# HeyWeCome/WhisprRec

Measured on AMD Instinct MI355X. Metric: BPR training triplets/sec, higher is better.
Workload: dtype f32; 1 GPU; BPRMF emb_size=64, synthetic 1000000 users x 1000000 items (uniform ids), batch 65536, SGD l2=0, plan build in timed region; batch=65536, emb_size=64, optimizer=SGD, plan_chunk_batches=64, tables=single GPU, step_stream=whisprrec_amd.hip_ops.PipelinedSgd, plan=group plan (no per-batch sort: flags + lists of the shared rows, wr_group.hip), chained_step_launch=True, plan_build=on a side stream, beside the steps of the chunk before

## Files before the change

whisprrec_amd/csrc/wr_group.hip:

```cpp
#include "wr_common.h"
#include <hip/hip_ext.h>

#include <algorithm>

namespace wr {

constexpr int kGpThreads = 1024;
constexpr unsigned kGpRangeBits = 18;
constexpr int kGpWords = 1 << (kGpRangeBits - 5);
constexpr int kGpCap = 8192;
constexpr int kGpBins = 4096;
constexpr int kGpMaxBin = 256;
constexpr int kGpMaxRanges = 8;
constexpr int64_t kGpMaxBatch = 1 << 17;
constexpr int kGpLongRun = 64;
constexpr int kGpMetaWords = 16;
#ifndef WR_GP_DBG
#define WR_GP_DBG 0
#endif

struct GroupLayout {
    int64_t nb, B, fw;
    int R_u, R_i, cap_u, cap_i;
    unsigned mask_u, mask_i, hbits_u, hbits_i;
    int64_t flags, ucnt, icnt, ul_row, ul_src, il_row, il_src, total;
    int64_t zero_words;
};

static inline int ranges_for(int64_t n_rows, unsigned *mask, unsigned *hbits, int *cap) {
    unsigned bits = kGpRangeBits;
    while (bits < kGpRangeBits + 3 && (int64_t(1) << bits) < n_rows) ++bits;
    *mask = (1u << bits) - 1u;
    *hbits = bits;
    const int R = 1 << (bits - kGpRangeBits);
    *cap = kGpCap;
    return R;
}

static bool group_layout(int64_t n, int64_t B, int64_t n_users, int64_t n_items, GroupLayout &L) {
    if (n <= 0 || n >= (int64_t(1) << 31) || B <= 0 || B > kGpMaxBatch) return false;
    if (n_users <= 0 || n_users >= (int64_t(1) << 31) || n_items <= 0 || n_items >= (int64_t(1) << 31)) return false;
    L.nb = (n + B - 1) / B;
    L.B = B;
    L.fw = (B + 31) / 32;
    L.R_u = ranges_for(n_users, &L.mask_u, &L.hbits_u, &L.cap_u);
    L.R_i = ranges_for(n_items, &L.mask_i, &L.hbits_i, &L.cap_i);
    L.flags = kGpMetaWords;
    L.ucnt = L.flags + L.nb * L.fw * 4;
    L.icnt = L.ucnt + align_up(L.nb * L.R_u, 4);
    L.zero_words = L.icnt + align_up(L.nb * L.R_i, 4);
    L.ul_row = L.zero_words;
    L.ul_src = L.ul_row + L.nb * L.R_u * (int64_t)L.cap_u;
    L.il_row = L.ul_src + L.nb * L.R_u * (int64_t)L.cap_u;
    L.il_src = L.il_row + L.nb * L.R_i * (int64_t)L.cap_i;
    L.total = L.il_src + L.nb * L.R_i * (int64_t)L.cap_i;
    return true;
}

struct GpDev {
    int *meta;
    unsigned *flags;
    int *ucnt, *icnt;
    int *ul_row, *ul_src, *il_row, *il_src;
    int R_u, R_i, cap_u, cap_i;
    unsigned mask_u, mask_i, hbits_u, hbits_i;
    int fw;
};

static inline GpDev group_dev(int32_t *plan, const GroupLayout &L) {
    return GpDev{plan, reinterpret_cast<unsigned *>(plan + L.flags), plan + L.ucnt, plan + L.icnt, plan + L.ul_row,
                 plan + L.ul_src, plan + L.il_row, plan + L.il_src, L.R_u, L.R_i, L.cap_u, L.cap_i, L.mask_u, L.mask_i,
                 L.hbits_u, L.hbits_i, (int)L.fw};
}

template <typename F>
__device__ __forceinline__ void gp_scan(const int *__restrict__ a, int cnt, F f) {
    if ((reinterpret_cast<uintptr_t>(a) & 15u) == 0) {
        const int n4 = cnt >> 2;
        const int4 *a4 = reinterpret_cast<const int4 *>(a);
        int i = threadIdx.x;
        for (; i + 3 * kGpThreads < n4; i += 4 * kGpThreads) {
            int4 v[4];
#pragma unroll
            for (int q = 0; q < 4; ++q) v[q] = a4[i + q * kGpThreads];
#pragma unroll
            for (int q = 0; q < 4; ++q) {
                const int at = 4 * (i + q * kGpThreads);
                f(v[q].x, at);
                f(v[q].y, at + 1);
                f(v[q].z, at + 2);
                f(v[q].w, at + 3);
            }
        }
        for (; i < n4; i += kGpThreads) {
            const int4 v = a4[i];
            f(v.x, 4 * i);
            f(v.y, 4 * i + 1);
            f(v.z, 4 * i + 2);
            f(v.w, 4 * i + 3);
        }
        for (int j = (n4 << 2) + threadIdx.x; j < cnt; j += kGpThreads) f(a[j], j);
    } else {
        for (int j = threadIdx.x; j < cnt; j += kGpThreads) f(a[j], j);
    }
}

__global__ __launch_bounds__(kGpThreads) void group_plan_kernel(const int *__restrict__ u, const int *__restrict__ p,
                                                                 const int *__restrict__ n, int64_t n_total, int B, int nb,
                                                                 int n_users, int n_items, GpDev L) {
    extern __shared__ __attribute__((aligned(16))) unsigned gp_lds[];
    unsigned *seen = gp_lds;
    unsigned long long *keys = reinterpret_cast<unsigned long long *>(gp_lds);
    unsigned *multi = gp_lds + 2 * kGpCap;
    unsigned *f0 = multi + kGpWords, *f1 = f0 + L.fw, *f2 = f1 + L.fw;
    int &n_list = *reinterpret_cast<int *>(f2 + L.fw);
    const int per = L.R_u + L.R_i;
    const unsigned lb = xcd_contiguous_id(blockIdx.x, gridDim.x);
    const int b = (int)(lb / (unsigned)per), rr = (int)(lb % (unsigned)per);
    const bool item = rr >= L.R_u;
    const unsigned r = (unsigned)(item ? rr - L.R_u : rr);
    const int64_t base = (int64_t)b * B;
    const int Bb = (int)((base + B <= n_total) ? B : (n_total - base));
    const unsigned n_rows = (unsigned)(item ? n_items : n_users);
    const unsigned mask = item ? L.mask_i : L.mask_u;
    const unsigned rb = (item ? L.hbits_i : L.hbits_u) - kGpRangeBits, rsel = (1u << rb) - 1u;
    for (int i = threadIdx.x; i < kGpWords; i += kGpThreads) {
        seen[i] = 0u;
        multi[i] = 0u;
    }
    for (int i = threadIdx.x; i < 3 * L.fw; i += kGpThreads) f0[i] = 0u;
    if (threadIdx.x == 0) n_list = 0;
    __syncthreads();
    auto mark = [&](int row, int) {
        if ((unsigned)row >= n_rows) {
            L.meta[0] = 1;
            return;
        }
        const unsigned h = (unsigned)row & mask;
        if ((h & rsel) != r) return;
        const unsigned bit = h >> rb, m = 1u << (bit & 31u);
        const unsigned old = atomicOr(&seen[bit >> 5], m);
        if (old & m) atomicOr(&multi[bit >> 5], m);
    };
    if (!(WR_GP_DBG & 8)) {
        if (item) {
            gp_scan(p + base, Bb, mark);
            gp_scan(n + base, Bb, mark);
        } else {
            gp_scan(u + base, Bb, mark);
        }
    }
    __syncthreads();
    auto several = [&](int row) -> bool {
        const unsigned h = (unsigned)row & mask;
        if ((h & rsel) != r) return false;
        const unsigned bit = h >> rb;
        return (multi[bit >> 5] >> (bit & 31u)) & 1u;
    };
    auto append = [&](int row, unsigned src) {
        const int pos = atomicAdd(&n_list, 1);
        if (pos < kGpCap) keys[pos] = ((unsigned long long)(unsigned)row << 32) | src;
    };
    if (!(WR_GP_DBG & 2)) {
        const bool next = b + 1 < nb && !(WR_GP_DBG & 16);
        const int64_t nbase = base + B;
        const int Bn = next ? (int)((nbase + B <= n_total) ? B : (n_total - nbase)) : 0;
        auto defer = [&](int row, int t) {
            if (several(row)) atomicOr(&f2[t >> 5], 1u << (t & 31));
        };
        if (item) {
            gp_scan(p + base, Bb, [&](int row, int t) {
                if (several(row)) {
                    atomicOr(&f0[t >> 5], 1u << (t & 31));
                    append(row, (unsigned)t << 1);
                }
            });
            gp_scan(n + base, Bb, [&](int row, int t) {
                if (several(row)) {
                    atomicOr(&f1[t >> 5], 1u << (t & 31));
                    append(row, ((unsigned)t << 1) | 1u);
                }
            });
            gp_scan(p + nbase, Bn, defer);
            gp_scan(n + nbase, Bn, defer);
        } else {
            gp_scan(u + base, Bb, [&](int row, int t) {
                if (several(row)) {
                    atomicOr(&f0[t >> 5], 1u << (t & 31));
                    append(row, (unsigned)t << 1);
                }
            });
            gp_scan(u + nbase, Bn, defer);
        }
    }
    __syncthreads();
    if (!(WR_GP_DBG & 4)) {
        unsigned *fb = L.flags + (int64_t)b * L.fw * 4;
        for (int w = threadIdx.x; w < L.fw; w += kGpThreads) {
            if (f0[w]) __hip_atomic_fetch_or(fb + 4 * w + (item ? 1 : 0), f0[w], __ATOMIC_RELAXED, __HIP_MEMORY_SCOPE_AGENT);
            if (item && f1[w]) __hip_atomic_fetch_or(fb + 4 * w + 2, f1[w], __ATOMIC_RELAXED, __HIP_MEMORY_SCOPE_AGENT);
            if (f2[w])
                __hip_atomic_fetch_or(fb + 4 * (L.fw + w) + 3, f2[w], __ATOMIC_RELAXED, __HIP_MEMORY_SCOPE_AGENT);
        }
    }
    const int cap = item ? L.cap_i : L.cap_u, R = item ? L.R_i : L.R_u;
    int m = n_list;
    if (m > cap) {
        if (threadIdx.x == 0) L.meta[1] = 1;
        m = cap;
    }
    int *cnt = reinterpret_cast<int *>(multi);
    unsigned short *out16 = reinterpret_cast<unsigned short *>(multi + kGpBins);
    int *wave_tot = reinterpret_cast<int *>(f0);
    auto bin_of = [&](unsigned long long k) -> int { return (int)(((((unsigned)(k >> 32)) & mask) >> rb) & (kGpBins - 1)); };
    int *lrow = (item ? L.il_row : L.ul_row) + ((int64_t)b * R + r) * cap, *lsrc = (item ? L.il_src : L.ul_src) + ((int64_t)b * R + r) * cap;
    __syncthreads();
    for (int i = threadIdx.x; i < kGpBins; i += kGpThreads) cnt[i] = 0;
    __syncthreads();
    if (!(WR_GP_DBG & 1)) {
        for (int j = threadIdx.x; j < m; j += kGpThreads) atomicAdd(&cnt[bin_of(keys[j])], 1);
        __syncthreads();
        constexpr int kOwn = kGpBins / kGpThreads;
        const int c0 = (int)threadIdx.x * kOwn;
        int local = 0;
#pragma unroll
        for (int j = 0; j < kOwn; ++j) local += cnt[c0 + j];
        int incl = local;
#pragma unroll
        for (int d = 1; d < 64; d <<= 1) {
            const int v = __shfl_up(incl, d, 64);
            if ((int)(threadIdx.x & 63) >= d) incl += v;
        }
        if ((threadIdx.x & 63) == 63) wave_tot[threadIdx.x >> 6] = incl;
        __syncthreads();
        int run = incl - local;
        for (int w = 0; w < (int)(threadIdx.x >> 6); ++w) run += wave_tot[w];
#pragma unroll
        for (int j = 0; j < kOwn; ++j) {
            const int c = cnt[c0 + j];
            cnt[c0 + j] = run;
            run += c;
        }
        __syncthreads();
        for (int j = threadIdx.x; j < m; j += kGpThreads) out16[atomicAdd(&cnt[bin_of(keys[j])], 1)] = (unsigned short)j;
        __syncthreads();
        for (int j = threadIdx.x; j < m; j += kGpThreads) {
            const unsigned long long k = keys[j];
            const int bin = bin_of(k);
            const int lo = bin ? cnt[bin - 1] : 0, hi = cnt[bin];
            if (hi - lo > kGpMaxBin) {
                L.meta[1] = 1;
                continue;
            }
            int pos = lo, same = 0;
            for (int jj = lo; jj < hi; ++jj) {
                const unsigned long long o = keys[out16[jj]];
                pos += o < k ? 1 : 0;
                same += (unsigned)(o >> 32) == (unsigned)(k >> 32) ? 1 : 0;
            }
            if (same > kGpLongRun) L.meta[2] = 1;
            lrow[pos] = (int)(k >> 32);
            lsrc[pos] = (int)(unsigned)k;
        }
    } else {
        for (int j = threadIdx.x; j < m; j += kGpThreads) {
            lrow[j] = (int)(keys[j] >> 32);
            lsrc[j] = (int)(unsigned)keys[j];
        }
    }
    if (threadIdx.x == 0) (item ? L.icnt : L.ucnt)[(int64_t)b * R + r] = m;
}

__global__ __launch_bounds__(kBlock) void narrow_ids_kernel(const int64_t *__restrict__ u, const int64_t *__restrict__ p,
                                                             const int64_t *__restrict__ n, int *__restrict__ u32,
                                                             int *__restrict__ p32, int *__restrict__ n32, int64_t cnt) {
    const int64_t i = (int64_t)blockIdx.x * kBlock + threadIdx.x;
    if (i >= cnt) return;
    const int64_t a = u[i], b = p[i], c = n[i];
    u32[i] = (a >= 0 && a < (int64_t(1) << 31)) ? (int)a : -1;
    p32[i] = (b >= 0 && b < (int64_t(1) << 31)) ? (int)b : -1;
    n32[i] = (c >= 0 && c < (int64_t(1) << 31)) ? (int)c : -1;
}

constexpr int kGsTile = 32;
constexpr int kGsAhead = 8;
constexpr int kGsShards = 64;
constexpr int kGsShardStride = 16;
constexpr int kGsStepWords = kGsShards * kGsShardStride;
constexpr int kGsDefChunk = 32;
constexpr int kGsLdsInts = 1024 + 8;
constexpr unsigned kGsSpinLimit = 1u << 22;

struct GsBatch {
    const int *u, *p, *n;
    const uint4 *flags;
    const int *ul_row, *ul_src, *ul_cnt, *il_row, *il_src, *il_cnt;
    int B, R_u, R_i, cap_u, cap_i;
};

struct GsArgs {
    float *U, *I;
    int D;
    float lr;
    GsBatch cur;
    float *Z, *ZU, *partials;
    float denom;
    GsBatch prev;
    const float *Zp, *ZUp, *partials_prev;
    int n_partials_prev;
    float denom_prev;
    float *loss_prev;
    int nA, nIT, nUT, nDS, tiles_at, side_at;
    int chained;
    unsigned *done, *timeout;
    float *Gs;
    int nL;
};

template <int NV>
__device__ __forceinline__ Row<NV> row_zero() {
    Row<NV> r;
#pragma unroll
    for (int k = 0; k < NV; ++k) r.v[k] = make_float4(0.f, 0.f, 0.f, 0.f);
    return r;
}

template <int T, int NV, bool FULL>
__device__ __forceinline__ void gs_single(const GsArgs &a, int t, int u, int p, int n, bool us, bool ps, bool ns, int lane,
                                          float &terms) {
    const Row<NV> ur = load_row<T, NV, FULL>(a.U, u, a.D, lane);
    const Row<NV> pr = load_row<T, NV, FULL>(a.I, p, a.D, lane);
    const Row<NV> nr = load_row<T, NV, FULL>(a.I, n, a.D, lane);
    const float sp = team_sum<T>(dot_partial<NV>(ur, pr));
    const float sn = team_sum<T>(dot_partial<NV>(ur, nr));
    float term, c;
    bpr_terms(sp, sn, a.denom, term, c);
    terms += term;
    Row<NV> g, z;
#pragma unroll
    for (int k = 0; k < NV; ++k) {
        g.v[k] = make_float4(c * (pr.v[k].x - nr.v[k].x), c * (pr.v[k].y - nr.v[k].y), c * (pr.v[k].z - nr.v[k].z),
                             c * (pr.v[k].w - nr.v[k].w));
        z.v[k] = make_float4(c * ur.v[k].x, c * ur.v[k].y, c * ur.v[k].z, c * ur.v[k].w);
    }
    const float lr = a.lr;
// ... 352 lines not shown
    TablePair tabs;
    const int32_t *u, *p, *n, *plan;
    int64_t n_triplets, batch_size, plan_words, workspace_bytes, sync_words;
    BatchRange range;
    float lr, *loss_out;
    void *const *events;
    void *workspace;
    uint32_t *sync;
    int n_cu;
    float *grad_slots;
    int64_t n_local_items, global_batch;
    hipStream_t stream;
};

template <int T, int NV, bool FULL>
static int32_t launch_group_steps(const GroupRun &g, const GroupLayout &L, const GpDev &G) {
    const int32_t D = g.tabs.D;
    const int64_t n_batches = g.range.n_batches, global_batch = g.global_batch;
    uint32_t *const sync = g.sync;
    const int64_t B = L.B;
    const int64_t ws_one = gs_ws_one(B, D), zb = align_up(B * (int64_t)D * 4, 256);
    char *ws = reinterpret_cast<char *>(g.workspace);
    float *Zs[2] = {reinterpret_cast<float *>(ws), reinterpret_cast<float *>(ws + ws_one)};
    float *ZUs[2] = {reinterpret_cast<float *>(ws + zb), reinterpret_cast<float *>(ws + ws_one + zb)};
    float *Ps[2] = {reinterpret_cast<float *>(ws + 2 * zb), reinterpret_cast<float *>(ws + ws_one + 2 * zb)};
    constexpr int TEAMS = kBlock / T;
    WR_HIP(hipMemsetAsync(sync, 0, (size_t)(n_batches * kGsStepWords) * 4, g.stream));
    uint32_t *timeout = sync + (g.sync_words - 4);
    int nDS = WR_GS_NDS;
    while (nDS > g.n_cu / 4 && nDS > 1) nDS >>= 1;
    auto batch_of = [&](int64_t b) {
        const int64_t off = b * B;
        const int Bk = (int)batch_len(g.n_triplets, B, b);
        return GsBatch{g.u + off, g.p + off, g.n + off, reinterpret_cast<const uint4 *>(G.flags + b * L.fw * 4),
                       G.ul_row + b * L.R_u * (int64_t)L.cap_u, G.ul_src + b * L.R_u * (int64_t)L.cap_u, G.ucnt + b * L.R_u,
                       G.il_row + b * L.R_i * (int64_t)L.cap_i, G.il_src + b * L.R_i * (int64_t)L.cap_i, G.icnt + b * L.R_i,
                       Bk, L.R_u, L.R_i, L.cap_u, L.cap_i};
    };
    auto ev = [&](int64_t k, int j) { return g.events ? reinterpret_cast<hipEvent_t>(g.events[2 * k + j]) : (hipEvent_t) nullptr; };
    int n_partials_prev = 0;
    for (int64_t k = 0; k <= n_batches; ++k) {
        GsArgs a{};
        a.U = g.tabs.U;
        a.I = g.tabs.I;
        a.D = D;
        a.lr = g.lr;
        a.done = sync + (k < n_batches ? k : 0) * kGsStepWords;
        a.timeout = timeout;
        a.Gs = g.grad_slots;
        a.nL = (int)g.n_local_items;
        const bool have_cur = k < n_batches, have_prev = k > 0;
        if (have_cur) {
            a.cur = batch_of(g.range.first_batch + k);
            a.Z = Zs[k & 1];
            a.ZU = ZUs[k & 1];
            a.partials = Ps[k & 1];
            a.denom = global_batch > 0 ? (float)global_batch : (float)a.cur.B;
            a.nA = (int)((a.cur.B + TEAMS - 1) / TEAMS);
            a.nDS = have_prev ? nDS : 0;
            a.chained = have_prev ? 1 : 0;
        }
        if (have_prev) {
            a.prev = batch_of(g.range.first_batch + k - 1);
            a.Zp = Zs[(k - 1) & 1];
            a.ZUp = ZUs[(k - 1) & 1];
            a.partials_prev = Ps[(k - 1) & 1];
            a.n_partials_prev = n_partials_prev;
            a.denom_prev = global_batch > 0 ? (float)global_batch : (float)a.prev.B;
            a.loss_prev = at_or_null(g.loss_out, k - 1);
            a.nIT = (int)std::min<int64_t>(WR_GS_NIT, (2 * B + kGsTile - 1) / kGsTile + L.R_i);
            a.nUT = (int)std::min<int64_t>(WR_GS_NUT, (B + kGsTile - 1) / kGsTile + L.R_u);
        }
        a.tiles_at = (int)((int64_t)a.nA * WR_GS_TILES_AT / 16);
        a.side_at = std::max(a.tiles_at, (int)((int64_t)a.nA * WR_GS_SIDE_AT / 16));
        const dim3 grid((unsigned)(a.nA + a.nIT + a.nUT + a.nDS));
        hipEvent_t e0 = have_cur ? ev(k, 0) : nullptr, e1 = have_cur ? ev(k, 1) : nullptr;
        if (e0 != nullptr || e1 != nullptr)
            hipExtLaunchKernelGGL((bprmf_group_step<T, NV, FULL>), grid, dim3(kBlock), 0, g.stream, e0, e1, 0, a);
        else
            hipLaunchKernelGGL((bprmf_group_step<T, NV, FULL>), grid, dim3(kBlock), 0, g.stream, a);
        WR_LAUNCH_CHECK("bprmf_group_step");
        n_partials_prev = a.nA + a.nDS;
    }
    return WR_OK;
}

static int32_t check_group_plan(const char *entry, const GroupRun &g, GroupLayout &L) {
    int32_t rc;
    if ((rc = check_whole_lines(entry, whole_lines(g.tabs.U, g.tabs.I, g.tabs.D), g.tabs.D)) != WR_OK) return rc;
    WR_REQUIRE(group_layout(g.n_triplets, g.batch_size, g.tabs.n_users, g.tabs.n_items, L), WR_E_RANGE,
               "group plan not applicable to n=%lld, batch=%lld", (long long)g.n_triplets, (long long)g.batch_size);
    WR_REQUIRE(g.plan_words >= L.total, WR_E_WORKSPACE, "group plan: %lld words < %lld", (long long)g.plan_words, (long long)L.total);
    return WR_OK;
}

static int32_t run_group(const char *entry, GroupRun &g, const GroupLayout &L, int64_t sync_batches) {
    int32_t rc;
    if ((rc = check_workspace(entry, g.workspace, g.workspace_bytes, 2 * gs_ws_one(g.batch_size, g.tabs.D))) != WR_OK) return rc;
    if ((rc = check_sync_words(entry, g.sync, g.sync_words, sync_batches * kGsStepWords + 4)) != WR_OK) return rc;
    if (g.range.n_batches == 0) return WR_OK;
    if (g.n_cu == 0 && (rc = device_cu_count(&g.n_cu)) != WR_OK) return rc;
    const GpDev G = group_dev(const_cast<int32_t *>(g.plan), L);
#define WR_CALL_GS(T_, NV_, FULL_) return launch_group_steps<T_, NV_, FULL_>(g, L, G)
    WR_DISPATCH_D(g.tabs.D, WR_CALL_GS);
#undef WR_CALL_GS
    return WR_OK;
}

}

using namespace wr;

extern "C" {

int64_t wr_group_plan_words(int64_t n_triplets, int64_t batch_size, int64_t n_users, int64_t n_items) {
    GroupLayout L;
    if (!group_layout(n_triplets, batch_size, n_users, n_items, L)) return 0;
    return L.total;
}

int32_t wr_group_plan_layout(int64_t n_triplets, int64_t batch_size, int64_t n_users, int64_t n_items, int64_t *out) {
    WR_REQUIRE(out != nullptr, WR_E_NULL, "out is NULL");
    GroupLayout L;
    WR_REQUIRE(group_layout(n_triplets, batch_size, n_users, n_items, L), WR_E_RANGE,
               "group plan not applicable to n=%lld, batch=%lld", (long long)n_triplets, (long long)batch_size);
    const int64_t v[16] = {L.nb, L.fw, L.R_u, L.R_i, (int64_t)L.mask_u, (int64_t)L.mask_i, L.flags, L.ucnt, L.icnt, L.ul_row,
                           L.ul_src, L.il_row, L.il_src, L.total, L.cap_u, L.cap_i};
    for (int i = 0; i < 16; ++i) out[i] = v[i];
    return WR_OK;
}

int32_t wr_narrow_ids_i64(const int64_t *u, const int64_t *p, const int64_t *n, int32_t *u32, int32_t *p32, int32_t *n32,
                          int64_t count, void *stream_) {
    WR_REQUIRE(u && p && n && u32 && p32 && n32, WR_E_NULL, "index arrays must not be NULL");
    WR_REQUIRE(count >= 0 && count < (int64_t(1) << 40), WR_E_SHAPE, "count out of range");
    if (count == 0) return WR_OK;
    hipLaunchKernelGGL(narrow_ids_kernel, dim3((unsigned)((count + kBlock - 1) / kBlock)), dim3(kBlock), 0,
                       reinterpret_cast<hipStream_t>(stream_), u, p, n, u32, p32, n32, count);
    WR_LAUNCH_CHECK("narrow_ids_kernel");
    return WR_OK;
}

int32_t wr_group_plan_build(const int32_t *u, const int32_t *p, const int32_t *n, int64_t n_triplets, int64_t batch_size,
                            int64_t n_users, int64_t n_items, int32_t *plan, int64_t plan_words, void *stream_) {
    WR_REQUIRE(u && p && n && plan, WR_E_NULL, "index arrays / plan must not be NULL");
    GroupLayout L;
    WR_REQUIRE(group_layout(n_triplets, batch_size, n_users, n_items, L), WR_E_RANGE,
               "group plan not applicable to n=%lld, batch=%lld", (long long)n_triplets, (long long)batch_size);
    WR_REQUIRE(aligned16(plan) && plan_words >= L.total, WR_E_WORKSPACE, "group plan: %lld words < %lld", (long long)plan_words,
               (long long)L.total);
    WR_REQUIRE(L.nb * (L.R_u + L.R_i) < (int64_t(1) << 31), WR_E_SHAPE, "group plan: too many batches in one plan");
    hipStream_t stream = reinterpret_cast<hipStream_t>(stream_);
    WR_HIP(hipMemsetAsync(plan, 0, (size_t)L.zero_words * 4, stream));
    const size_t lds = (size_t)(2 * kGpCap + kGpWords + 3 * L.fw + 4) * 4;
    static bool attr_set = false;
    if (!attr_set) {
        WR_HIP(hipFuncSetAttribute(reinterpret_cast<const void *>(group_plan_kernel), hipFuncAttributeMaxDynamicSharedMemorySize,
                                   (int)((2 * kGpCap + kGpWords + 3 * ((kGpMaxBatch + 31) / 32) + 4) * 4)));
        attr_set = true;
    }
    const GpDev G = group_dev(plan, L);
    hipLaunchKernelGGL(group_plan_kernel, dim3((unsigned)(L.nb * (L.R_u + L.R_i))), dim3(kGpThreads), lds, stream, u, p, n,
                       n_triplets, (int)batch_size, (int)L.nb, (int)n_users, (int)n_items, G);
    WR_LAUNCH_CHECK("group_plan_kernel");
    return WR_OK;
}

int64_t wr_bprmf_group_workspace_bytes(int64_t batch_size, int32_t D) { return 2 * gs_ws_one(batch_size, D); }

int64_t wr_bprmf_group_sync_words(int64_t n_batches) { return n_batches < 0 ? WR_E_SHAPE : (n_batches + 1) * kGsStepWords + 4; }

int32_t wr_bprmf_group_supported(const float *user_tab, const float *item_tab, int32_t D) {
    return (user_tab && item_tab && D >= 4 && D <= 1024 && D % 4 == 0 && whole_lines(user_tab, item_tab, D)) ? 1 : 0;
}

int32_t wr_bprmf_run_sgd_group(float *user_tab, int64_t n_users, float *item_tab, int64_t n_items, int32_t D,
                               const int32_t *u, const int32_t *p, const int32_t *n, int64_t n_triplets, int64_t batch_size,
                               const int32_t *plan, int64_t plan_words, int64_t first_batch, int64_t n_batches, float lr,
                               float *loss_out, void *const *events, void *workspace, int64_t workspace_bytes, int32_t *sync,
                               int64_t sync_words, void *stream) {
    GroupRun g{};
    g.tabs = TablePair{user_tab, item_tab, n_users, n_items, D};
    g.u = u; g.p = p; g.n = n; g.n_triplets = n_triplets; g.batch_size = batch_size;
    g.plan = plan; g.plan_words = plan_words;
    g.range = BatchRange{first_batch, n_batches};
    g.lr = lr; g.loss_out = loss_out; g.events = events;
    g.workspace = workspace; g.workspace_bytes = workspace_bytes;
    g.sync = reinterpret_cast<uint32_t *>(sync); g.sync_words = sync_words;
    g.stream = reinterpret_cast<hipStream_t>(stream);
    int32_t rc;
    GroupLayout L;
    if ((rc = check_tables(g.tabs)) != WR_OK) return rc;
    WR_REQUIRE(u && p && n && plan && sync, WR_E_NULL, "index arrays / plan / sync words must not be NULL");
    if ((rc = check_group_plan("wr_bprmf_run_sgd_group", g, L)) != WR_OK) return rc;
    WR_REQUIRE(first_batch >= 0 && n_batches >= 0 && first_batch + n_batches <= L.nb, WR_E_SHAPE,
               "batches [%lld,%lld) exceed the plan's %lld", (long long)first_batch, (long long)(first_batch + n_batches),
               (long long)L.nb);
    return run_group("wr_bprmf_run_sgd_group", g, L, n_batches + 1);
}

int32_t wr_bprmf_shard_step_group(float *user_shard, int64_t n_user_rows, float *item_ext, int64_t n_ext_rows,
                                  int64_t n_local_items, int32_t D, const int32_t *vu, const int32_t *vp, const int32_t *vn,
                                  int64_t n_triplets, int64_t batch_size, const int32_t *plan, int64_t plan_words, int64_t batch,
                                  int64_t global_batch, float lr, float *grad_slots, float *loss_partial, void *workspace,
                                  int64_t workspace_bytes, int32_t *sync, int64_t sync_words, void *stream) {
    GroupRun g{};
    g.tabs = TablePair{user_shard, item_ext, n_user_rows, n_ext_rows, D};
    g.u = vu; g.p = vp; g.n = vn; g.n_triplets = n_triplets; g.batch_size = batch_size;
    g.plan = plan; g.plan_words = plan_words;
    g.range = BatchRange{batch, 1};
    g.lr = lr; g.loss_out = loss_partial;
    g.workspace = workspace; g.workspace_bytes = workspace_bytes;
    g.sync = reinterpret_cast<uint32_t *>(sync); g.sync_words = sync_words;
    g.n_cu = 256;
    g.grad_slots = grad_slots; g.n_local_items = n_local_items; g.global_batch = global_batch;
    g.stream = reinterpret_cast<hipStream_t>(stream);
    int32_t rc;
    GroupLayout L;
    if ((rc = check_tables(g.tabs, "user_shard", "item_ext")) != WR_OK) return rc;
    WR_REQUIRE(vu && vp && vn && plan && sync && grad_slots, WR_E_NULL, "index arrays / plan / sync words / grad_slots must not be NULL");
    WR_REQUIRE(aligned16(grad_slots), WR_E_ALIGN, "grad_slots is not 16-byte aligned");
    WR_REQUIRE(n_local_items >= 0 && n_local_items <= n_ext_rows, WR_E_SHAPE, "n_local_items %lld outside [0, %lld]",
               (long long)n_local_items, (long long)n_ext_rows);
    if ((rc = check_group_plan("wr_bprmf_shard_step_group", g, L)) != WR_OK) return rc;
    WR_REQUIRE(batch >= 0 && batch < L.nb, WR_E_SHAPE, "batch %lld outside the plan's %lld", (long long)batch, (long long)L.nb);
    WR_REQUIRE(global_batch >= batch_size, WR_E_SHAPE, "global_batch %lld < local batch %lld", (long long)global_batch,
               (long long)batch_size);
    return run_group("wr_bprmf_shard_step_group", g, L, 2);
}

}
```

whisprrec_amd/hip_ops.py:

```python
import ctypes

import torch

from . import abi


def _stream():
    return torch.cuda.current_stream().cuda_stream


def _p(t):
    return None if t is None else t.data_ptr()


def _addr(struct):
    return ctypes.addressof(struct) if struct is not None else None


def _event_handles(events, per_step, count, allow_none):
    if events is None:
        return None
    if len(events) != per_step * count:
        raise ValueError("%s must hold %d events per step" % ("phase_events" if per_step == 4 else "events", per_step))
    handles = []
# ... 1043 lines not shown

def sgd_dense(tab, grad, lr, l2=0.0, stamp=None, step_id=0):
    abi.check(abi.lib().wr_sgd_dense(_p(_req(tab, torch.float32, "tab", 2)), tab.shape[0], tab.shape[1],
                                     _p(_req(grad, torch.float32, "grad", 2)), _p(stamp), step_id, lr, l2, _stream()),
              "wr_sgd_dense")


def adam_dense(tab, exp_avg, exp_avg_sq, grad, adam_step, lr, l2=0.0, beta1=0.9, beta2=0.999, eps=1e-8, stamp=None,
               step_id=0):
    for t, nm in ((tab, "tab"), (exp_avg, "exp_avg"), (exp_avg_sq, "exp_avg_sq"), (grad, "grad")):
        _req(t, torch.float32, nm, 2)
    abi.check(abi.lib().wr_adam_dense(_p(tab), _p(exp_avg), _p(exp_avg_sq), tab.shape[0], tab.shape[1], _p(grad),
                                      _p(stamp), step_id, adam_step, lr, l2, beta1, beta2, eps, _stream()),
              "wr_adam_dense")


def _join_views(ts):
    if len(ts) == 1:
        return ts[0]
    a = ts[0]
    adjacent, end = a.is_contiguous(), a.storage_offset() + a.numel()
    for b in ts[1:]:
        adjacent = adjacent and b.is_contiguous() and b.dtype == a.dtype and \
            b.untyped_storage().data_ptr() == a.untyped_storage().data_ptr() and b.storage_offset() == end
        end += b.numel()
    if adjacent:
        return torch.as_strided(a, (end - a.storage_offset(),), (1,), a.storage_offset())
    return torch.cat(ts)


class PipelinedSgd:

    PREFETCH_AFTER_TRIPLETS = 0
    PLAN_TRIPLETS = 1 << 22
    GROUP_MIN_ROWS_PER_TRIPLET = 12
    GROUP_MIN_BATCH = 4096

    CHAIN_MIN_BATCH = 8192
    CHAIN_MIN_ITEMS_PER_TRIPLET = 6

    def __init__(self, chunk=64, min_triplets=None, chain=True, inline_plan=False, group=True):
        import sys
        self.ops = sys.modules[__name__]
        self.chunk = int(chunk)
        self.chain = bool(chain)
        self.group = bool(group)
        self.inline_plan = inline_plan
        self.stats = {"plain_calls": 0, "chain_calls": 0, "group_calls": 0, "group_fallbacks": 0}
        self._garenas = {}
        if min_triplets is not None:
            self.PLAN_TRIPLETS = int(min_triplets)
        self.plan_stream = None
        self._arenas = {}

    def chunk_batches(self, batch_size):
        return max(self.chunk, self.PLAN_TRIPLETS // max(int(batch_size), 1))

    def _arena_pair(self, device, B, nb_total, overlap_items):
        cap = min(self.chunk_batches(B), max(int(nb_total), 1)) * B
        key = (str(device), B, int(overlap_items))
        pair = self._arenas.get(key)
        if pair is None or pair[0].max_triplets < cap:
            pair = [self.ops.PlanArena(device, cap, B, overlap_items=overlap_items) for _ in range(2)]
            self._arenas[key] = pair
        return pair

    def _garena_pair(self, device, B, nb_total, n_users, n_items):
        cap = min(self.chunk_batches(B), max(int(nb_total), 1)) * B
        key = (str(device), B, int(n_users), int(n_items))
        pair = self._garenas.get(key)
        if pair is None or pair[0].max_triplets < cap:
            pair = [self.ops.GroupArena(device, cap, B, n_users, n_items) for _ in range(2)]
            self._garenas[key] = pair
        return pair

    def plan(self, U, segments, batch, first_chunk=None, lr=None, prep=None, runner=None):
        if self.plan_stream is None:
            self.plan_stream = side_stream(U.device)
        B = int(batch)
        segs, first = [], 0
        for k, (rows, u, p, n) in enumerate(segments):
            nb = (u.numel() + B - 1) // B
            if u.numel() % B != 0 and any(s[1].numel() for s in segments[k + 1:]):
                raise ValueError("only the last segment may end with a short batch")
            segs.append({"tabs": self.ops.BprmfTables(U, rows) if nb else None, "nb": nb, "first": first})
            first += nb
        live = [s for s in segments if s[1].numel()]
        u_all, p_all, n_all = (_join_views([s[j] for s in live]) for j in (1, 2, 3))
        n_items = max([s[0].shape[0] for s in live] or [1])
        main = torch.cuda.current_stream(U.device)
        use_chain = self.chain and (runner is None or getattr(runner, "wants_chain_marks", False)) and \
            B >= self.CHAIN_MIN_BATCH and first >= 2 and \
            min([s[0].shape[0] for s in live] or [0]) >= self.CHAIN_MIN_ITEMS_PER_TRIPLET * B and \
            all(sg["tabs"].chain_supported() for sg in segs if sg["tabs"] is not None)
        min_rows = min([U.shape[0]] + [s[0].shape[0] for s in live])
        use_group = self.group and runner is None and len(live) == 1 and first >= 2 and \
            self.GROUP_MIN_BATCH <= B <= 131072 and u_all.dtype in (torch.int32, torch.int64) and \
            min_rows >= self.GROUP_MIN_ROWS_PER_TRIPLET * B and \
            all(sg["tabs"].group_supported() for sg in segs if sg["tabs"] is not None)
        garenas = self._garena_pair(U.device, B, first, U.shape[0], n_items) if use_group else None
        arenas = None if use_group else self._arena_pair(U.device, B, first, n_items if use_chain else 0)
        for a in (arenas or []) + (garenas or []):
            a.release_after(main)
        h = {"segs": segs, "B": B, "u": u_all, "p": p_all, "n": n_all, "nb": first, "n_users": U.shape[0], "n_items": n_items,
             "at": 0, "tag": 0, "next": None, "cur": None, "map": None, "arenas": arenas, "pos": 0,
             "group": use_group, "garenas": garenas, "device": U.device,
             "ids32": [torch.empty(u_all.numel(), dtype=torch.int32, device=U.device) for _ in range(3)]
                      if use_group and u_all.dtype == torch.int64 else None,
             "chain": use_chain, "prep": prep, "runner": runner, "inline": bool(self.inline_plan),
             "lead": [int(c) for c in (first_chunk if isinstance(first_chunk, (list, tuple)) else [first_chunk or 0]) if c]}
        self.plan_stream.wait_stream(main)
        self._prefetch(h)
        return h

    def _build_stream(self, h):
        return torch.cuda.current_stream(h["u"].device) if h["inline"] else self.plan_stream

    def _prefetch(self, h):
        if h["at"] >= h["nb"]:
            h["next"] = None
            return
        first, B = h["at"], h["B"]
        c = min(self.chunk_batches(B), h["nb"] - first)
        if h["lead"]:
            c = min(c, h["lead"].pop(0))
        h["at"] += c
        lo, hi = first * B, min(h["u"].numel(), (first + c) * B)
        with torch.cuda.stream(self._build_stream(h)):
            bmap = h["map"] if h["map"] else None
            if h["prep"] is not None:
                h["prep"].fill(lo, hi)
            if h["group"]:
                cols = (h["u"], h["p"], h["n"])
                if h["ids32"] is not None:
                    abi.check(abi.lib().wr_narrow_ids_i64(*[_p(c[lo:hi]) for c in cols], *[_p(c[lo:hi]) for c in h["ids32"]],
                                                          hi - lo, _stream()), "wr_narrow_ids_i64")
                    cols = h["ids32"]
                plan = self.ops.GroupPlan(cols[0][lo:hi], cols[1][lo:hi], cols[2][lo:hi], B, h["n_users"], h["n_items"],
                                          arena=h["garenas"][h["tag"]], defer=True)
                h["tag"] ^= 1
                h["next"] = (first, plan)
                return
            if h["arenas"] is None:
                h["arenas"] = self._arena_pair(h["device"], B, h["nb"], h["n_items"] if h["chain"] else 0)
            plan = self.ops.BatchPlan(h["u"][lo:hi], h["p"][lo:hi], h["n"][lo:hi], B, h["n_users"], h["n_items"],
                                      validate=False, ws_tag="rot%d" % h["tag"], bucket_map=bmap, arena=h["arenas"][h["tag"]],
                                      defer=True, overlap=h["chain"])
        h["tag"] ^= 1
        h["next"] = (first, plan)

    STICKY_MSG = "a wait inside a step launch expired (hand-off between the workgroups of one launch): the tables are not " \
                 "valid — do not save or evaluate them; restart the run"

    def _queue_sticky(self, h, tabs, main):
        words = tabs.sticky_words()
        if not words:
            return
        pin = h.get("sticky_pin")
        if pin is None or pin.numel() < 2 * len(words):
            pin = h["sticky_pin"] = torch.zeros(2 * max(len(words), 4), dtype=torch.int32, pin_memory=True)
        half = pin.numel() // 2
        off = half * (h.get("sticky_tag", 0) & 1)
        h["sticky_tag"] = h.get("sticky_tag", 0) + 1
        for j, wd in enumerate(words):
            pin[off + j:off + j + 1].copy_(wd, non_blocking=True)
        ev = torch.cuda.Event()
        ev.record(main)
        self._check_sticky(h)
        h["sticky_pending"] = (ev, pin[off:off + len(words)])

    def _check_sticky(self, h):
        pend = h.pop("sticky_pending", None)
        if pend is not None:
            pend[0].synchronize()
            if bool(pend[1].numpy().any()):
                raise abi.WhisprRecHipError(self.STICKY_MSG)

    def _take_next(self, h, pos, main):
        self._check_sticky(h)
        if h["next"] is None:
            self._prefetch(h)
        cur = h["next"]
        assert cur is not None and cur[0] == pos, "steps must be run in order"
        plan = cur[1]
        plan.validate()
        if isinstance(plan, GroupPlan):
            if plan.overflow or plan.long_run:
                h["group"] = False
                self.stats["group_fallbacks"] += 1
                if h["next"] is not None and h["next"][0] != cur[0]:
                    raise AssertionError("plan pipeline out of step")
                if plan.overflow:
                    first, B = cur[0], h["B"]
                    lo, hi = first * B, first * B + plan.n_triplets
                    plan.arena.release_after(main)
                    if h["arenas"] is None:
                        h["arenas"] = self._arena_pair(h["device"], B, h["nb"], h["n_items"] if h["chain"] else 0)
                    with torch.cuda.stream(self._build_stream(h)):
                        plan = self.ops.BatchPlan(h["u"][lo:hi], h["p"][lo:hi], h["n"][lo:hi], B, h["n_users"], h["n_items"],
                                                  validate=False, ws_tag="rot%d" % h["tag"], arena=h["arenas"][h["tag"]],
                                                  defer=True, overlap=h["chain"])
                    h["tag"] ^= 1
                    plan.validate()
                    cur = (first, plan)
            main.wait_event(plan.ready)
            h["cur"], h["next"] = cur, None
            return cur
        main.wait_event(plan.ready)
        if plan.fast_overflowed:
            if plan._mapped():
                h["map"] = False
            elif h["map"] is None:
                with torch.cuda.stream(self._build_stream(h)):
                    src = (h["prep"].users, h["prep"].items) if h["prep"] is not None else (h["u"], h["p"])
                    h["map"] = self.ops.BucketMap(src[0], src[1], h["n_users"], h["n_items"], h["B"])
        if h["chain"] and plan.hot is not None:
            h["chain"] = False
        if h["chain"] and plan.hot is None and plan.overlap is not None and not plan.overlap["fits"]:
            dcn = plan.overlap["def_count_np"]
            if int((dcn[1:] > plan.overlap["cap"]).sum()) * 2 > plan.n_batches - 1:
                h["chain"] = False
        h["cur"], h["next"] = cur, None
        return cur

    def _run_span(self, h, sg, pos, end, lr, losses, loss_off):
        main = torch.cuda.current_stream(sg["tabs"].U.device)
        while pos < end:
            cur = h["cur"]
            if cur is None or pos >= cur[0] + cur[1].n_batches:
                cur = self._take_next(h, pos, main)
            base, plan = cur
            c = min(end, base + plan.n_batches) - pos
            if h["inline"] and h["next"] is None and h["at"] < h["nb"]:
                mid = base + plan.n_batches // 2
                if pos >= mid:
                    self._prefetch(h)
                else:
                    c = min(c, mid - pos)
            elif self.PREFETCH_AFTER_TRIPLETS > 0 and h["next"] is None and h["at"] < h["nb"] and \
                    c > (self.PREFETCH_AFTER_TRIPLETS + h["B"] - 1) // h["B"]:
                c = (self.PREFETCH_AFTER_TRIPLETS + h["B"] - 1) // h["B"]
            if isinstance(plan, GroupPlan):
                sg["tabs"].run_sgd_group(plan, pos - base, c, lr, losses=losses[loss_off:loss_off + c])
                self.stats["group_calls"] += 1
            elif h["runner"] is not None:
                h["runner"](plan, pos - base, c, losses[loss_off:loss_off + c])
                self.stats["plain_calls"] += 1
            elif h["chain"] and plan.overlap is not None and c >= 2:
                sg["tabs"].run_sgd_chain(plan, pos - base, c, lr, losses=losses[loss_off:loss_off + c])
                self.stats["chain_calls"] += 1
            else:
                sg["tabs"].run_sgd(plan, pos - base, c, lr, losses=losses[loss_off:loss_off + c])
                self.stats["plain_calls"] += 1
            pos += c
            loss_off += c
            if pos >= base + plan.n_batches:
                plan.arena.release_after(main)
                self._queue_sticky(h, sg["tabs"], main)
            if h["next"] is None and not h["inline"]:
                self._prefetch(h)
        h["pos"] = pos

    def run(self, handle, seg, lr, losses):
        sg = handle["segs"][seg]
        if sg["nb"] == 0:
            return
        self._run_span(handle, sg, sg["first"], sg["first"] + sg["nb"], lr, losses, 0)
        if seg == len(handle["segs"]) - 1:
            self._check_sticky(handle)

    def run_steps(self, handle, count, lr, losses):
        assert len(handle["segs"]) == 1, "run_steps: single-segment handles"
        sg = handle["segs"][0]
        pos = handle["pos"]
        if pos + count > sg["nb"]:
            raise ValueError("run_steps: %d steps asked, %d left" % (count, sg["nb"] - pos))
        self._run_span(handle, sg, pos, pos + count, lr, losses, 0)


class LazyOptimizerState:

    FOLD_MAX_GAP = 40

    MAX_LAG = 64
    LAG_MIN_GAP = 64

    def __init__(self, tabs, name, lr, l2, betas=(0.9, 0.999), eps=1e-8, fold=None, max_lag=None):
        self.chain, self.chain_calls = True, 0
        if name not in ("SGD", "Adam"):
            raise ValueError(name)
        self.tabs, self.name, self.lr, self.l2, self.betas, self.eps = tabs, name, float(lr), float(l2), betas, float(eps)
        self.fold = fold if fold is None else bool(fold)
        self.max_lag = max_lag if max_lag is None else int(max_lag)
        self._sweep_pos = (ctypes.c_int64 * 2)(0, 0)
        dev = tabs.dev
        self.t = 0
        self.flushed_at = 0
        self.last_u = torch.zeros(tabs.U.shape[0], dtype=torch.int32, device=dev)
        self.last_i = torch.zeros(tabs.I.shape[0], dtype=torch.int32, device=dev)
        if name == "Adam":
            z = torch.zeros_like
            self.m_u, self.v_u, self.m_i, self.v_i = z(tabs.U), z(tabs.U), z(tabs.I), z(tabs.I)
            self.consts = None
            self._grow_consts(4096)

    def _folds(self, plan):
        if self.fold is None:
            gap = max(self.tabs.U.shape[0], self.tabs.I.shape[0]) / float(max(plan.batch_size, 1))
            return gap <= self.FOLD_MAX_GAP
        return self.fold

    def _adam_state(self):
        return (_p(self.m_u), _p(self.v_u), _p(self.m_i), _p(self.v_i), _p(self.last_u), _p(self.last_i))

    def _grow_consts(self, n):
        host = torch.empty(2 * n, dtype=torch.float32)
        abi.check(abi.lib().wr_adam_consts(0, n, self.lr, self.betas[0], self.betas[1], host.data_ptr()), "wr_adam_consts")
        self.consts = host.to(self.tabs.dev)
        self.n_consts = n

    def _adam_rows(self, tab, m, v, last, keys_ptr, n_keys, grad):
        abi.check(abi.lib().wr_adam_rows_lazy(_p(tab), _p(m), _p(v), _p(last), tab.shape[0], tab.shape[1], keys_ptr, n_keys,
                                              _p(grad), self.t, _p(self.consts), self.n_consts, self.l2, self.betas[0],
                                              self.betas[1], self.eps, _stream()), "wr_adam_rows_lazy")

    def step(self, plan, k, loss_out=None):
        tabs = self.tabs
        if _auto_lag(self, plan) > 0 and not (self.name == "Adam" and self._folds(plan)):
            out = self.run(plan, k, 1, losses=None if loss_out is None else loss_out.reshape(1))
            return out.reshape(()) if loss_out is None else loss_out
        self.t += 1
        batch = tabs._plan_ptrs(plan, k)
        tu, oi, B = batch[0], batch[3], batch[5]
        if self.name == "Adam":
            if self.t >= self.n_consts:
                self._grow_consts(2 * self.n_consts)
            hot = plan.hot_struct(k)
            folded = self._folds(plan) and hot is None
            if not folded:
                self._adam_rows(tabs.U, self.m_u, self.v_u, self.last_u, tu, B, None)
                self._adam_rows(tabs.I, self.m_i, self.v_i, self.last_i, oi, 2 * B, None)
            loss_out = tabs._loss_buf(loss_out)
            ws = tabs._ws(plan.batch_size)
            head = (*tabs._table_head(), *self._adam_state(), *batch, self.t, self.lr)
            tail = (self.l2, self.betas[0], self.betas[1], self.eps, _p(loss_out))
            if folded:
                abi.check(abi.lib().wr_bprmf_step_adam_folded(*head, _p(self.consts), self.n_consts, *tail, _p(ws), ws.numel(),
                                                              _stream()), "wr_bprmf_step_adam_folded")
            else:
                abi.check(abi.lib().wr_bprmf_step_adam(*head, *tail, _addr(hot), _p(ws), ws.numel(), _stream()),
                          "wr_bprmf_step_adam")
            tabs.step_id += 1
            return loss_out
        L = abi.lib()
        for tab, last, keys, n in ((tabs.U, self.last_u, tu, B), (tabs.I, self.last_i, oi, 2 * B)):
            abi.check(L.wr_sgd_rows_lazy(_p(tab), _p(last), tab.shape[0], tab.shape[1], keys, n, self.t, self.lr, self.l2,
                                         _stream()), "wr_sgd_rows_lazy")
        return tabs.step_sgd(plan, k, self.lr, self.l2, loss_out=loss_out, decay_untouched=False)

    def run(self, plan, first, count, losses=None):
        tabs, L = self.tabs, abi.lib()
        losses = tabs._loss_buf(losses, count)
        ws = tabs._ws(plan.batch_size)
        su, si = tabs._stamps()
        hot = plan.hot_struct()
        t0 = self.t + 1
        lag = _auto_lag(self, plan)
        if self.name == "Adam":
            while self.t + count >= self.n_consts:
                self._grow_consts(2 * self.n_consts)
            head = (*tabs._table_head(), *self._adam_state(), *tabs._plan_head(plan), first, count, t0, self.lr,
                    _p(self.consts), self.n_consts, self.l2, self.betas[0], self.betas[1], self.eps, _p(losses), _addr(hot))
            o = getattr(plan, "overlap", None)
            if self._folds(plan) and self.chain and o is not None and hot is None and count >= 2 and tabs.chain_supported():
                ws2 = tabs.overlap_workspace(plan.batch_size)
                sync = tabs._chain_sync(count)
                abi.check(L.wr_bprmf_run_adam_folded_chain(*head[:-1], _p(o["tdef"]), _p(o["def_q"]),
                                                           o["def_count_host"].data_ptr(), o["cap"], o["cap"], _p(ws2),
                                                           ws2.numel(), _p(sync), sync.numel(), _stream()),
                          "wr_bprmf_run_adam_folded_chain")
                self.chain_calls += 1
            elif self._folds(plan):
                abi.check(L.wr_bprmf_run_adam_folded(*head, _p(ws), ws.numel(), _stream()), "wr_bprmf_run_adam_folded")
            elif lag > 0:
                abi.check(L.wr_bprmf_run_adam_lazy_bounded(*head, lag, _addr(self._sweep_pos), _p(ws), ws.numel(), _stream()),
                          "wr_bprmf_run_adam_lazy_bounded")
            else:
                abi.check(L.wr_bprmf_run_adam_lazy(*head, _p(ws), ws.numel(), _stream()), "wr_bprmf_run_adam_lazy")
        else:
            head = (*tabs._table_head(), _p(self.last_u), _p(self.last_i), _p(su), _p(si), tabs.step_id + 1,
                    *tabs._plan_head(plan), first, count, t0, self.lr, self.l2, _p(losses), _addr(hot))
            if lag > 0:
                abi.check(L.wr_bprmf_run_sgd_lazy_bounded(*head, lag, _addr(self._sweep_pos), _p(ws), ws.numel(), _stream()),
                          "wr_bprmf_run_sgd_lazy_bounded")
            else:
                abi.check(L.wr_bprmf_run_sgd_lazy(*head, _p(ws), ws.numel(), _stream()), "wr_bprmf_run_sgd_lazy")
        self.t += count
        tabs.step_id += count
        return losses

    def flush(self):
        if self.flushed_at == self.t:
            return
        L, tabs = abi.lib(), self.tabs
        if self.name == "Adam":
            for tab, m, v, last in ((tabs.U, self.m_u, self.v_u, self.last_u), (tabs.I, self.m_i, self.v_i, self.last_i)):
                abi.check(L.wr_adam_catchup_all(_p(tab), _p(m), _p(v), _p(last), *tab.shape, self.t, _p(self.consts),
                                                self.n_consts, self.l2, self.betas[0], self.betas[1], self.eps, _stream()),
                          "wr_adam_catchup_all")
        else:
            for tab, last in ((tabs.U, self.last_u), (tabs.I, self.last_i)):
                abi.check(L.wr_sgd_catchup_all(_p(tab), _p(last), *tab.shape, self.t, self.lr, self.l2, _stream()),
                          "wr_sgd_catchup_all")
        self.flushed_at = self.t


class StatefulSparseState:

    KIND = {"Adagrad": 1, "Adadelta": 2}

    MAX_LAG, LAG_MIN_GAP = 64, 64

    def __init__(self, tabs, name, lr, rho=0.9, eps=None, max_lag=None):
        if name not in self.KIND:
            raise ValueError(name)
        self.max_lag = max_lag if max_lag is None else int(max_lag)
        self._sweep_pos = (ctypes.c_int64 * 2)(0, 0)
        self.tabs, self.name, self.lr, self.rho = tabs, name, float(lr), float(rho)
        self.eps = float(eps) if eps is not None else (1e-10 if name == "Adagrad" else 1e-6)
        z = torch.zeros_like
# ... 339 lines not shown
```

Before: 2.585 billion triplets/s.

## Interleave column scans in group plan kernel and lag sticky-word host checks

The group-plan kernel now scans all columns (pos/neg of this and the next batch) in one loop that keeps a fixed number of int4 loads in flight across columns. Before, each column was scanned in a separate pass. The aim is more memory-level parallelism and fewer loop passes, at the cost of clamped redundant loads and a more complex edge-handling path. On the host, the sticky-error check now lets up to two pending copies stay outstanding before it synchronizes, so the CPU blocks on the GPU less often per chunk. Error detection is delayed by one extra step.

```diff
diff --git a/whisprrec_amd/csrc/wr_group.hip b/whisprrec_amd/csrc/wr_group.hip
--- a/whisprrec_amd/csrc/wr_group.hip
+++ b/whisprrec_amd/csrc/wr_group.hip
@@ -5,7 +5,13 @@
 
 namespace wr {
 
-constexpr int kGpThreads = 1024;
+#ifndef WR_GP_THREADS
+#define WR_GP_THREADS 1024
+#endif
+#ifndef WR_GP_IN_FLIGHT
+#define WR_GP_IN_FLIGHT 8
+#endif
+constexpr int kGpThreads = WR_GP_THREADS;
 constexpr unsigned kGpRangeBits = 18;
 constexpr int kGpWords = 1 << (kGpRangeBits - 5);
 constexpr int kGpCap = 8192;
@@ -73,35 +79,67 @@
                  L.hbits_u, L.hbits_i, (int)L.fw};
 }
 
-template <typename F>
-__device__ __forceinline__ void gp_scan(const int *__restrict__ a, int cnt, F f) {
-    if ((reinterpret_cast<uintptr_t>(a) & 15u) == 0) {
-        const int n4 = cnt >> 2;
-        const int4 *a4 = reinterpret_cast<const int4 *>(a);
-        int i = threadIdx.x;
-        for (; i + 3 * kGpThreads < n4; i += 4 * kGpThreads) {
-            int4 v[4];
-#pragma unroll
-            for (int q = 0; q < 4; ++q) v[q] = a4[i + q * kGpThreads];
-#pragma unroll
-            for (int q = 0; q < 4; ++q) {
-                const int at = 4 * (i + q * kGpThreads);
-                f(v[q].x, at);
-                f(v[q].y, at + 1);
-                f(v[q].z, at + 2);
-                f(v[q].w, at + 3);
-            }
-        }
-        for (; i < n4; i += kGpThreads) {
-            const int4 v = a4[i];
-            f(v.x, 4 * i);
-            f(v.y, 4 * i + 1);
-            f(v.z, 4 * i + 2);
-            f(v.w, 4 * i + 3);
-        }
-        for (int j = (n4 << 2) + threadIdx.x; j < cnt; j += kGpThreads) f(a[j], j);
-    } else {
-        for (int j = threadIdx.x; j < cnt; j += kGpThreads) f(a[j], j);
+constexpr int kGpInFlight = WR_GP_IN_FLIGHT;
+
+template <int NC, typename F>
+__device__ __forceinline__ void gp_visit(const int *const (&col)[NC], const int (&cnt)[NC], F f) {
+    constexpr int Q = kGpInFlight / NC;
+    static_assert(Q >= 1 && Q * NC == kGpInFlight, "columns of a visit share the loads in flight evenly");
+    const int4 *a4[NC], *full = nullptr;
+    int head[NC], n4[NC], most = 0;
+    bool edges = false;
+#pragma unroll
+    for (int c = 0; c < NC; ++c) {
+        const int lead = (int)((16u - (unsigned)(reinterpret_cast<uintptr_t>(col[c]) & 15u)) & 15u) >> 2;
+        head[c] = lead < cnt[c] ? lead : cnt[c];
+        a4[c] = reinterpret_cast<const int4 *>(col[c] + head[c]);
+        n4[c] = (cnt[c] - head[c]) >> 2;
+        if (n4[c] > most) {
+            most = n4[c];
+            full = a4[c];
+        }
+        edges = edges || 4 * n4[c] != cnt[c];
+    }
+#pragma unroll
+    for (int c = 0; c < NC; ++c)
+        if (n4[c] == 0) a4[c] = full;
+    for (int i0 = threadIdx.x; i0 < most; i0 += Q * kGpThreads) {
+        int4 v[NC][Q];
+#pragma unroll
+        for (int q = 0; q < Q; ++q) {
+#pragma unroll
+            for (int c = 0; c < NC; ++c) {
+                const int i = i0 + q * kGpThreads, last = n4[c] > 0 ? n4[c] - 1 : 0;
+                v[c][q] = a4[c][i < last ? i : last];
+            }
+        }
+#pragma unroll
+        for (int q = 0; q < Q; ++q) {
+#pragma unroll
+            for (int c = 0; c < NC; ++c) {
+                const int i = i0 + q * kGpThreads;
+                if (i < n4[c]) {
+                    const int at = head[c] + 4 * i;
+                    f(c, v[c][q].x, at);
+                    f(c, v[c][q].y, at + 1);
+                    f(c, v[c][q].z, at + 2);
+                    f(c, v[c][q].w, at + 3);
+                }
+            }
+        }
+    }
+    if (edges) {
+        int edge_at[NC], edge[NC];
+#pragma unroll
+        for (int c = 0; c < NC; ++c) {
+            const int t = (int)threadIdx.x;
+            edge_at[c] = t < head[c] ? t : 4 * n4[c] + t;
+            if (edge_at[c] >= cnt[c]) edge_at[c] = -1;
+            edge[c] = (cnt[c] > 0 ? col[c] : col[0])[edge_at[c] >= 0 ? edge_at[c] : 0];
+        }
+#pragma unroll
+        for (int c = 0; c < NC; ++c)
+            if (edge_at[c] >= 0) f(c, edge[c], edge_at[c]);
     }
 }
 
@@ -131,7 +169,7 @@
     for (int i = threadIdx.x; i < 3 * L.fw; i += kGpThreads) f0[i] = 0u;
     if (threadIdx.x == 0) n_list = 0;
     __syncthreads();
-    auto mark = [&](int row, int) {
+    auto mark = [&](int, int row, int) {
         if ((unsigned)row >= n_rows) {
             L.meta[0] = 1;
             return;
@@ -144,10 +182,13 @@
     };
     if (!(WR_GP_DBG & 8)) {
         if (item) {
-            gp_scan(p + base, Bb, mark);
-            gp_scan(n + base, Bb, mark);
+            const int *const col[2] = {p + base, n + base};
+            const int len[2] = {Bb, Bb};
+            gp_visit<2>(col, len, mark);
         } else {
-            gp_scan(u + base, Bb, mark);
+            const int *const col[1] = {u + base};
+            const int len[1] = {Bb};
+            gp_visit<1>(col, len, mark);
         }
     }
     __syncthreads();
@@ -165,32 +206,30 @@
         const bool next = b + 1 < nb && !(WR_GP_DBG & 16);
         const int64_t nbase = base + B;
         const int Bn = next ? (int)((nbase + B <= n_total) ? B : (n_total - nbase)) : 0;
+        auto share = [&](unsigned *fl, int row, int t, unsigned neg) {
+            if (several(row)) {
+                atomicOr(&fl[t >> 5], 1u << (t & 31));
+                append(row, ((unsigned)t << 1) | neg);
+            }
+        };
         auto defer = [&](int row, int t) {
             if (several(row)) atomicOr(&f2[t >> 5], 1u << (t & 31));
         };
         if (item) {
-            gp_scan(p + base, Bb, [&](int row, int t) {
-                if (several(row)) {
-                    atomicOr(&f0[t >> 5], 1u << (t & 31));
-                    append(row, (unsigned)t << 1);
-                }
+            const int *const col[4] = {p + base, n + base, p + nbase, n + nbase};
+            const int len[4] = {Bb, Bb, Bn, Bn};
+            gp_visit<4>(col, len, [&](int c, int row, int t) {
+                if (c == 0) share(f0, row, t, 0u);
+                else if (c == 1) share(f1, row, t, 1u);
+                else defer(row, t);
             });
-            gp_scan(n + base, Bb, [&](int row, int t) {
-                if (several(row)) {
-                    atomicOr(&f1[t >> 5], 1u << (t & 31));
-                    append(row, ((unsigned)t << 1) | 1u);
-                }
+        } else {
+            const int *const col[2] = {u + base, u + nbase};
+            const int len[2] = {Bb, Bn};
+            gp_visit<2>(col, len, [&](int c, int row, int t) {
+                if (c == 0) share(f0, row, t, 0u);
+                else defer(row, t);
             });
-            gp_scan(p + nbase, Bn, defer);
-            gp_scan(n + nbase, Bn, defer);
-        } else {
-            gp_scan(u + base, Bb, [&](int row, int t) {
-                if (several(row)) {
-                    atomicOr(&f0[t >> 5], 1u << (t & 31));
-                    append(row, (unsigned)t << 1);
-                }
-            });
-            gp_scan(u + nbase, Bn, defer);
         }
     }
     __syncthreads();
@@ -849,7 +888,7 @@
     WR_REQUIRE(L.nb * (L.R_u + L.R_i) < (int64_t(1) << 31), WR_E_SHAPE, "group plan: too many batches in one plan");
     hipStream_t stream = reinterpret_cast<hipStream_t>(stream_);
     WR_HIP(hipMemsetAsync(plan, 0, (size_t)L.zero_words * 4, stream));
-    const size_t lds = (size_t)(2 * kGpCap + kGpWords + 3 * L.fw + 4) * 4;
+    const size_t lds = (size_t)(2 * kGpCap + kGpWords + std::max<int64_t>(3 * L.fw + 4, 64)) * 4;
     static bool attr_set = false;
     if (!attr_set) {
         WR_HIP(hipFuncSetAttribute(reinterpret_cast<const void *>(group_plan_kernel), hipFuncAttributeMaxDynamicSharedMemorySize,
diff --git a/whisprrec_amd/hip_ops.py b/whisprrec_amd/hip_ops.py
--- a/whisprrec_amd/hip_ops.py
+++ b/whisprrec_amd/hip_ops.py
@@ -1219,32 +1219,40 @@
     STICKY_MSG = "a wait inside a step launch expired (hand-off between the workgroups of one launch): the tables are not " \
                  "valid — do not save or evaluate them; restart the run"
 
+    STICKY_LAG = 2
+
     def _queue_sticky(self, h, tabs, main):
         words = tabs.sticky_words()
         if not words:
             return
+        self._check_sticky(h, keep=self.STICKY_LAG - 1)
+        h.setdefault("sticky_pending", []).append(self._sticky_copy(h, words, main))
+
+    def _sticky_copy(self, h, words, main):
+        slots = self.STICKY_LAG + 1
         pin = h.get("sticky_pin")
-        if pin is None or pin.numel() < 2 * len(words):
-            pin = h["sticky_pin"] = torch.zeros(2 * max(len(words), 4), dtype=torch.int32, pin_memory=True)
-        half = pin.numel() // 2
-        off = half * (h.get("sticky_tag", 0) & 1)
+        if pin is None or pin.numel() < slots * len(words):
+            self._check_sticky(h)
+            pin = h["sticky_pin"] = torch.zeros(slots * max(len(words), 4), dtype=torch.int32, pin_memory=True)
+        part = pin.numel() // slots
+        off = part * (h.get("sticky_tag", 0) % slots)
         h["sticky_tag"] = h.get("sticky_tag", 0) + 1
         for j, wd in enumerate(words):
             pin[off + j:off + j + 1].copy_(wd, non_blocking=True)
         ev = torch.cuda.Event()
         ev.record(main)
-        self._check_sticky(h)
-        h["sticky_pending"] = (ev, pin[off:off + len(words)])
-
-    def _check_sticky(self, h):
-        pend = h.pop("sticky_pending", None)
-        if pend is not None:
-            pend[0].synchronize()
-            if bool(pend[1].numpy().any()):
+        return ev, pin[off:off + len(words)]
+
+    def _check_sticky(self, h, keep=0):
+        pend = h.get("sticky_pending")
+        while pend and len(pend) > keep:
+            ev, words = pend.pop(0)
+            ev.synchronize()
+            if bool(words.numpy().any()):
                 raise abi.WhisprRecHipError(self.STICKY_MSG)
 
     def _take_next(self, h, pos, main):
-        self._check_sticky(h)
+        self._check_sticky(h, keep=self.STICKY_LAG - 1)
         if h["next"] is None:
             self._prefetch(h)
         cur = h["next"]
@@ -1343,6 +1351,8 @@
         if pos + count > sg["nb"]:
             raise ValueError("run_steps: %d steps asked, %d left" % (count, sg["nb"] - pos))
         self._run_span(handle, sg, pos, pos + count, lr, losses, 0)
+        if handle["pos"] >= sg["nb"]:
+            self._check_sticky(handle)
 
 
 class LazyOptimizerState:
```

After: 2.592 billion triplets/s (median of 6 runs). No clear change (+0.3%).
